# lauradarcy/gym-craftingworld

Measured on AMD Instinct MI355X. Metric: env-steps/sec at 65536 envs, 1/2/4/8 MI355X; bit-exact vs CPU ref, higher is better.
Workload: dtype u8; 1 GPU; BASELINE configs[2]: 65536 envs/GPU, 21x21 grid, full-frame 4x4-cell uint8 pixel obs, auto-reset, uniform random actions, max_steps=300; envs_per_gpu=65536, size=21, max_steps=300, obs_mode=pixels, raster=ray, task_lists=one (all nine tasks), launch=eager, episode_phases=synchronized start

## Files before the change

### gym_craftingworld_amd/csrc/cw_kernels.hip

```cpp
#include <hip/hip_runtime.h>
#include <stdint.h>

#include "cw_layout.h"
#include "cw_mt.h"

#define CW_WAVE 64
#define CW_BALLOT(p) __builtin_amdgcn_ballot_w64(p)
#define CW_ALT_FRAME_PACE 2

#ifdef CW_TRACE
__device__ unsigned long long cw_trace_buf[1024 * 8];
#define CW_STAMP(env, k) do { if (lane == 0) { cw_trace_buf[((env) & 1023) * 8 + (k)] = wall_clock64(); \
                                               if ((k) == 0 || (k) == 5) cw_trace_buf[((env) & 1023) * 8 + 6 + ((k) ? 1 : 0)] = clock64(); } } while (0)
extern "C" hipError_t cwk_trace_read(unsigned long long *dst) { return hipMemcpyFromSymbol(dst, HIP_SYMBOL(cw_trace_buf), sizeof(cw_trace_buf)); }
#else
#define CW_STAMP(env, k) do { } while (0)
#endif

enum { EMPTY = 0, STICKS = 1, AXE = 2, HAMMER = 3, ROCK = 4, TREE = 5, BREAD = 6, HOUSE = 7, WHEAT = 8 };
enum { T_MAKEBREAD = 0, T_EATBREAD = 1, T_BUILDHOUSE = 2, T_CHOPTREE = 3, T_CHOPROCK = 4,
       T_GOTOHOUSE = 5, T_MOVEAXE = 6, T_MOVEHAMMER = 7, T_MOVESTICKS = 8 };

typedef uint32_t u32x3 __attribute__((ext_vector_type(3)));
typedef u32x3 u32x3_a4 __attribute__((aligned(4)));
// ... 105 lines not shown
                                                bool whole)
{
    const uint32_t row_bytes = 9u * S;
    uint8_t *p = frame + (size_t)(3u * S) * row_bytes;
    if (whole) {
        for (uint32_t b = first; b < 3u * row_bytes; b += step) {
            const uint32_t x = b % row_bytes;
            p[b] = (hold != 0 && x >= 9u && x < 18u) ? 255 : 0;
        }
    } else {
        for (uint32_t j = first; j < 27u; j += step) p[(j / 9u) * row_bytes + 9u + (j % 9u)] = hold ? 255 : 0;
    }
}
__device__ __forceinline__ void render_frame_alt(uint8_t *__restrict__ dst0, uint8_t *__restrict__ dst1, int S, int ncell,
                                                 uint32_t div_magic, const uint32_t sp[8], uint32_t codes,
                                                 uint32_t agent_cell, uint32_t hold, int lane, int pace)
{
    const uint32_t row_bytes = 9u * S, FB = 27u * S * (uint32_t)(S + 1);
    uint32_t pos = 0xFFFFFFFFu, item = 0;
#pragma unroll
    for (int q = 0; q < 8; q++) {
        pos = (lane == q) ? sp[q] : pos;
        item = (lane == q) ? ((codes >> (4 * q)) & 15u) : item;
    }
    if (lane == 8) { pos = agent_cell; item = 9u; }
    if (lane == 9) { pos = agent_cell; item = hold; }
    uint32_t p_off = 0xFFFFFFFFu, p_val = 0;
    if (lane < 10 && item != 0 && pos < (uint32_t)ncell) {
        const uint32_t r = __umulhi(pos, div_magic), c = pos - r * S, k = item - 1u;
        const uint32_t k3 = (k >= 6u) ? 2u : (k >= 3u) ? 1u : 0u;
        p_off = (3u * r + k3) * row_bytes + 9u * c + 3u * (k - 3u * k3);
        p_val = cpv_color((int)k);
    } else if (lane >= 10 && lane < 19 && hold != 0) {
        const uint32_t j = (uint32_t)lane - 10u, jr = (j >= 6u) ? 2u : (j >= 3u) ? 1u : 0u;
        p_off = (3u * S + jr) * row_bytes + 9u + 3u * (j - 3u * jr);
        p_val = 0x00FFFFFFu;
    }
    const uint32_t held_off = __builtin_amdgcn_readlane(p_off, 9);
    const bool twice = lane < 8 && p_off != 0xFFFFFFFFu && p_off == held_off;
    if (twice) p_val = ((2u * (p_val & 0xFFu)) & 0xFFu) | ((2u * (p_val & 0xFF00u)) & 0xFF00u) | ((2u * (p_val & 0xFF0000u)) & 0xFF0000u);
    if (CW_BALLOT(twice) && lane == 9) p_off = 0xFFFFFFFFu;
    const bool p_any = p_off != 0xFFFFFFFFu;
    for (int which = 0; which < 2; which++) {
        uint8_t *const dst = which ? dst1 : dst0;
        if (!dst) break;
        const uint32_t head = (uint32_t)(-(intptr_t)dst) & 15u;
        const uint32_t n_body = (FB - head) >> 4;
        const uint32_t tail0 = head + 16u * n_body;
        if ((uint32_t)lane < head) dst[lane] = 0;
        if (tail0 + (uint32_t)lane < FB) dst[tail0 + lane] = 0;
        for (uint32_t j = (uint32_t)lane; j < n_body; j += CW_WAVE) {
            *(uint4 *)(dst + head + 16u * j) = make_uint4(0, 0, 0, 0);
            for (int z = 0; z < pace; z++) __builtin_amdgcn_s_sleep(1);
        }
        if (p_any) {
            dst[p_off] = (uint8_t)p_val;
            dst[p_off + 1] = (uint8_t)(p_val >> 8);
            dst[p_off + 2] = (uint8_t)(p_val >> 16);
        }
    }
}

__device__ __forceinline__ void render_frame(uint8_t *__restrict__ dst0, uint8_t *__restrict__ dst1,
                                             int S, int ncell, uint32_t div_magic, const uint32_t sp[8],
                                             const uint32_t rgb[8], uint32_t agent_cell, uint32_t hold_rgb,
                                             int lane)
{
    const uint32_t row_bytes = 12u * S;
    for (uint32_t cell = lane; cell < (uint32_t)ncell; cell += CW_WAVE) {
        const uint32_t r = __umulhi(cell, div_magic);
        const uint32_t c = cell - r * S;
        uint32_t col = 0;
#pragma unroll
        for (int k = 0; k < 8; k++) col = (cell == sp[k]) ? rgb[k] : col;
        const u32x3 d = cell_row_dwords(col);
        const bool ag = (cell == agent_cell);
        const u32x3 d1 = ag ? overlay_dwords(d, 0x00FFFFFFu) : d;
        const u32x3 d2 = ag ? overlay_dwords(d, hold_rgb) : d;
        const size_t off = (size_t)(4u * r) * row_bytes + 12u * c;
        uint8_t *q = dst0 + off;
        *(u32x3_a4 *)(q) = d;
        *(u32x3_a4 *)(q + row_bytes) = d1;
        *(u32x3_a4 *)(q + 2 * row_bytes) = d2;
        *(u32x3_a4 *)(q + 3 * row_bytes) = d;
        if (dst1) {
            uint8_t *q1 = dst1 + off;
            *(u32x3_a4 *)(q1) = d;
            *(u32x3_a4 *)(q1 + row_bytes) = d1;
            *(u32x3_a4 *)(q1 + 2 * row_bytes) = d2;
            *(u32x3_a4 *)(q1 + 3 * row_bytes) = d;
        }
    }
}
__device__ __forceinline__ void paint_state_frame(const CwParams &P, uint8_t *dst, const uint32_t sp[8], uint32_t codes, uint32_t agent_cell,
                                                  uint32_t hold, int lane, uint8_t *dst1 = nullptr)
{
    if (P.raster == 1) {
        render_frame_alt(dst, dst1, P.size, P.ncell, P.div_magic, sp, codes, agent_cell, hold, lane, CW_ALT_FRAME_PACE);
    } else {
        uint32_t rgb[8];
#pragma unroll
        for (int k = 0; k < 8; k++) rgb[k] = rgb_of_code((codes >> (4 * k)) & 15u);
        render_frame(dst, dst1, P.size, P.ncell, P.div_magic, sp, rgb, agent_cell, hold ? rgb_of_code(hold) : 0x00FFFFFFu, lane);
    }
}
__device__ __forceinline__ uint32_t agent_cell_of(const CwParams &P, uint32_t hx) { return (hx & 0xFFu) * P.size + ((hx >> 8) & 0xFFu); }
__device__ __forceinline__ uint32_t hold_of(uint32_t hx) { return (hx >> 16) & 0xFFu; }
enum { CW_SRC_CURRENT = 0, CW_SRC_INIT = 1, CW_SRC_GOAL = 2 };
__device__ __forceinline__ void load_state_uniform(const CwParams &P, int env, int src, uint32_t sp[8], uint32_t &codes, uint32_t &agent_cell, uint32_t &hold)
{
    uint4 v_p;
    uint32_t v_c, v_a, v_h = 0;
    if (src == CW_SRC_CURRENT) {
        const uint4 h = P.hdr[env];
        v_p = P.pos[env];
        v_c = h.w;
        v_a = agent_cell_of(P, h.x);
        v_h = hold_of(h.x);
    } else if (src == CW_SRC_INIT) {
        v_p = P.init_pos[env];
        v_c = CW_CODES_INITIAL;
        v_a = P.init_agent[env];
    } else {
        v_p = P.goal_pos[env];
        v_c = P.goal_codes[env];
        v_a = P.goal_agent[env];
    }
    unpack_pos(make_uint4(__builtin_amdgcn_readfirstlane(v_p.x), __builtin_amdgcn_readfirstlane(v_p.y), __builtin_amdgcn_readfirstlane(v_p.z),
                          __builtin_amdgcn_readfirstlane(v_p.w)), sp);
    codes = __builtin_amdgcn_readfirstlane(v_c);
    agent_cell = __builtin_amdgcn_readfirstlane(v_a);
    hold = __builtin_amdgcn_readfirstlane(v_h);
}

struct CwStepOut {
    int reward;
    bool done, success, invalid, changed;
    uint32_t dirty0, dirty1;
    bool mark0, mark1;
    uint32_t step_num, achieved, desired;
    uint32_t n_success;
};

__device__ __forceinline__ int32_t episode_return_of(const CwParams &P, const CwStepOut &o)
{
    return (int32_t)o.n_success * (P.max_steps + 1) - (int32_t)o.step_num;
}

template <typename InitPosFn>
__device__ __forceinline__ CwStepOut step_env(const CwParams &P, uint4 &h, uint32_t sp[8], int a, InitPosFn load_init_pos)
{
    CwStepOut o;
    const int S = P.size;
    int ar = h.x & 0xFF, ac = (h.x >> 8) & 0xFF;
    uint32_t hold = (h.x >> 16) & 0xFF;
    uint32_t achieved = h.y & 0xFFFFu;
    const uint32_t desired = h.y >> 16;
    const uint32_t step_num = min((h.z & 0xFFFFu) + 1u, 0xFFFFu);
    const uint32_t flags = (h.z >> 16) & ~CW_FLAG_RESET;
    uint32_t codes = h.w;

    o.invalid = (unsigned)a > 5u;
    bool changed = false;
    const uint32_t cell = ar * S + ac;
    const int idx_here = slot_at(sp, cell);
    const uint32_t code_here = code_of(codes, idx_here);
    o.dirty0 = cell;
    o.dirty1 = 0xFFFFFFFFu;
    o.mark0 = o.mark1 = false;

    if (a == 4) {
        if (code_here >= STICKS && code_here <= HAMMER && hold == 0) {
            hold = code_here;
#pragma unroll
            for (int k = 0; k < 8; k++) sp[k] = (k == idx_here) ? CW_POS_HELD : sp[k];
            changed = true;
        }
    } else if (a == 5) {
        if (hold != 0 && idx_here < 0) {
#pragma unroll
            for (int k = 0; k < 8; k++) sp[k] = (sp[k] == CW_POS_HELD) ? cell : sp[k];
            hold = 0;
            changed = true;
        }
    } else if (!o.invalid) {
        const int dr = (a == 0) ? -1 : (a == 2) ? 1 : 0;
        const int dc = (a == 1) ? 1 : (a == 3) ? -1 : 0;
        const int nr = min(max(ar + dr, 0), S - 1);
        const int nc = min(max(ac + dc, 0), S - 1);
        uint32_t old_obj = 0;
        uint32_t cur_code = code_here;
        if (nr != ar || nc != ac) {
            const uint32_t ncell = nr * S + nc;
            const int idx_t = slot_at(sp, ncell);
            const uint32_t t = code_of(codes, idx_t);
            const bool cant = (t == ROCK && hold != 3) || (t == TREE && hold != 2);
            if (!cant) {
                changed = true;
                o.dirty1 = ncell;
                o.mark0 = true;
                ar = nr; ac = nc;
                old_obj = t;
                uint32_t nw = t;
                if (t == ROCK || t == BREAD) nw = EMPTY;
                else if (t == TREE) nw = STICKS;
                else if (t == STICKS && hold == 3) nw = HOUSE;
                else if (t == WHEAT && hold == 2) nw = BREAD;
                if (nw != t) {
                    codes = (codes & ~(15u << (4 * idx_t))) | (nw << (4 * idx_t));
                    if (nw == EMPTY) {
#pragma unroll
                        for (int k = 0; k < 8; k++) sp[k] = (k == idx_t) ? CW_POS_GONE : sp[k];
                    }
                }
                cur_code = nw;
                o.mark1 = nw == t;
            }
        }
        const uint32_t pcell = ar * S + ac;
        if (old_obj == BREAD) achieved |= 1u << T_EATBREAD;
        else if (old_obj == ROCK) achieved |= 1u << T_CHOPROCK;
        else if (old_obj == TREE) achieved |= 1u << T_CHOPTREE;
        achieved = (cur_code == HOUSE) ? (achieved | (1u << T_GOTOHOUSE))
                                       : (achieved & ~(1u << T_GOTOHOUSE));
        if (hold != 0) {
            const uint4 ip = load_init_pos();
            const uint32_t ip_sticks = ip.x & 0xFFFFu, ip_axe = ip.x >> 16;
            const uint32_t ip_hammer = ip.y & 0xFFFFu, ip_tree = ip.z & 0xFFFFu;
            if (hold == 1) {
                const bool home = (pcell == ip_sticks) ||
                                  (pcell == ip_tree && (achieved & (1u << T_CHOPTREE)));
                achieved = home ? (achieved & ~(1u << T_MOVESTICKS)) : (achieved | (1u << T_MOVESTICKS));
            } else if (hold == 2) {
                if (old_obj == WHEAT) achieved |= 1u << T_MAKEBREAD;
                achieved = (pcell == ip_axe) ? (achieved & ~(1u << T_MOVEAXE)) : (achieved | (1u << T_MOVEAXE));
            } else {
                if (old_obj == STICKS) achieved |= 1u << T_BUILDHOUSE;
                achieved = (pcell == ip_hammer) ? (achieved & ~(1u << T_MOVEHAMMER)) : (achieved | (1u << T_MOVEHAMMER));
            }
        }
    }

    int reward = -1;
    if (changed) {
        const uint32_t am = achieved & P.task_mask, dm = desired & P.task_mask;
        bool hit;
        if (flags & CW_FLAG_SUBSET)
            hit = ((dm & ~am) == 0) && (((~(dm ^ am)) & P.task_mask) != 0);
        else
            hit = (am == dm);
        reward = hit ? P.max_steps : -1;
    }
    o.reward = reward;
    o.changed = changed;
    o.success = (reward == P.max_steps);
    o.done = (step_num >= (uint32_t)P.max_steps) || o.success;
    o.step_num = step_num;
    o.achieved = achieved;
    o.desired = desired;
    o.n_success = min((flags >> 2) + (o.success ? 1u : 0u), 0x3FFFu);

    h.x = (uint32_t)ar | ((uint32_t)ac << 8) | (hold << 16) | (h.x & 0xFF000000u);
    h.y = achieved | (desired << 16);
    h.z = step_num | (((flags & 3u) | (o.n_success << 2)) << 16);
    h.w = codes;
    return o;
}

__device__ __forceinline__ void paint_changed_cells(const CwParams &P, int env, const uint4 &h, const uint32_t sp[8], const CwStepOut &o)
{
    uint8_t *frame = P.obs + (size_t)env * P.frame_bytes;
    const uint32_t hold = hold_of(h.x);
    const uint32_t acell = agent_cell_of(P, h.x);
    if (P.raster == 1) {
        const uint32_t r0 = __umulhi(o.dirty0, P.div_magic);
        alt_paint_tile(frame, P.size, r0, o.dirty0 - r0 * P.size, code_of(h.w, slot_at(sp, o.dirty0)), o.dirty0 == acell, hold);
        if (o.dirty1 != 0xFFFFFFFFu) {
            const uint32_t r1 = __umulhi(o.dirty1, P.div_magic);
            alt_paint_tile(frame, P.size, r1, o.dirty1 - r1 * P.size, code_of(h.w, slot_at(sp, o.dirty1)), o.dirty1 == acell, hold);
        }
        alt_paint_strip(frame, P.size, hold, 0, 1, false);
    } else {
        paint_cell(frame, P.size, o.dirty0, code_of(h.w, slot_at(sp, o.dirty0)), o.dirty0 == acell, hold, P.div_magic, o.mark0);
        if (o.dirty1 != 0xFFFFFFFFu)
            paint_cell(frame, P.size, o.dirty1, code_of(h.w, slot_at(sp, o.dirty1)), o.dirty1 == acell, hold, P.div_magic, o.mark1);
    }
}

__device__ __forceinline__ void store_step_outputs(const CwParams &P, int env, const CwStepOut &o)
{
    P.reward[env] = o.reward;
    P.done[env] = o.done ? 1 : 0;
    P.achieved_out[env] = (uint16_t)o.achieved;
    P.desired_out[env] = (uint16_t)o.desired;
    if (o.done) { P.episode_length[env] = (int32_t)o.step_num; P.episode_return[env] = episode_return_of(P, o); }
}

__device__ __forceinline__ int load_action(const void *actions, int act_dtype, int i)
{
    if (act_dtype == 0) return ((const int32_t *)actions)[i];
    if (act_dtype == 1) { const long long a = ((const long long *)actions)[i]; return a == (long long)(int)a ? (int)a : -1; }
    return ((const uint8_t *)actions)[i];
}

struct CwGoalState { uint4 pos; uint32_t codes, agent; };
__device__ __forceinline__ bool pop_next_episode(const CwParams &P, int env, uint32_t ctl, uint4 &h, uint32_t sp[8], bool count_episode, CwGoalState *goal = nullptr)
{
    const uint32_t slot = ctl & 0xFFu;
    const size_t at = (size_t)slot * P.n_envs + env;
    const uint4 m = P.nx_misc[at];
    const uint4 ipos = P.nx_init_pos[at];
    const uint4 gpos = P.nx_goal_pos[at];
    const int32_t ep_no = count_episode ? P.ep_no[env] : 0;
    if (!(m.z >> 31)) return false;
    P.init_pos[env] = ipos;
    P.goal_pos[env] = gpos;
    if (goal) { goal->pos = gpos; goal->codes = m.y; goal->agent = m.x >> 16; }
    P.goal_codes[env] = m.y;
    P.init_agent[env] = (uint16_t)(m.x & 0xFFFFu);
    P.goal_agent[env] = (uint16_t)(m.x >> 16);
    if (count_episode) P.ep_no[env] = ep_no + 1;
    ((uint32_t *)(P.nx_misc + at))[2] = 0;
    P.nx_ctl[env] = (slot + 1u == CW_LA_DEPTH ? 0u : slot + 1u) | CW_CTL_QUEUED;
    const uint32_t ia = m.x & 0xFFFFu;
    const uint32_t ar = __umulhi(ia, P.div_magic), ac = ia - ar * P.size;
    h.x = ar | (ac << 8) | (h.x & 0xFF000000u);
    h.y = (m.z & 0xFFFFu) << 16;
    h.z = (CW_FLAG_RESET | (((m.z >> 16) & 1u) ? CW_FLAG_SUBSET : 0u)) << 16;
    h.w = CW_CODES_INITIAL;
    unpack_pos(ipos, sp);
    return true;
}

__device__ __forceinline__ void note_slow_reset(const CwParams &P, int env, uint32_t ctl)
{
    atomicAdd(&P.counters[5], 1ull);
    if (!(ctl & CW_CTL_QUEUED)) P.nx_ctl[env] = ctl | CW_CTL_QUEUED;
}

__global__ __launch_bounds__(256) void cw_step_kernel(CwParams P, const void *actions, int act_dtype, int paint_dirty)
{
    const int i = blockIdx.x * blockDim.x + threadIdx.x;
    if (i == 0) {
        atomicAdd(&P.counters[0], (unsigned long long)P.n_envs);
    }
    const bool live = i < P.n_envs;
    bool done = false, success = false, invalid = false;
    if (live) {
        const int a = load_action(actions, act_dtype, i);
        uint4 h = P.hdr[i];
        uint32_t sp[8];
        unpack_pos(P.pos[i], sp);
        const CwStepOut o = step_env(P, h, sp, a, [&]() { return P.init_pos[i]; });
        done = o.done; success = o.success; invalid = o.invalid;

        P.hdr[i] = h;
        P.pos[i] = pack_pos(sp);
        store_step_outputs(P, i, o);
        if (paint_dirty && o.changed) paint_changed_cells(P, i, h, sp, o);
    }
    const unsigned long long m_done = CW_BALLOT(done), m_succ = CW_BALLOT(success), m_inv = CW_BALLOT(invalid);
    if ((m_done | m_inv) && (threadIdx.x & (CW_WAVE - 1)) == 0) {
        if (m_done) atomicAdd(&P.counters[1], (unsigned long long)__popcll(m_done));
        if (m_succ) atomicAdd(&P.counters[2], (unsigned long long)__popcll(m_succ));
        if (m_inv) atomicAdd(&P.counters[3], (unsigned long long)__popcll(m_inv));
    }
}


__device__ __forceinline__ uint32_t shuffle_tokens(CwMtWave &mt, int n)
{
    const uint32_t lane = mt.lane;
    uint32_t hit = 0;
    uint32_t v_tok = 0;
    int i = n - 1;

    while (i >= 10) {
        if (mt.used == 64) mt.gen();
        const int take = min(64 - mt.used, i - 8);
        const uint32_t d = mt.v_out;
        const unsigned long long valid = (~0ull >> (64 - take)) << mt.used;
        unsigned long long acc = CW_BALLOT((d & (0xFFFFFFFFu >> __builtin_clz((uint32_t)i))) <= (uint32_t)i) & valid;
        uint32_t i_l = 0, v_l = 0;
        for (;;) {
            const uint32_t before = __builtin_amdgcn_mbcnt_hi((uint32_t)(acc >> 32),
                                                              __builtin_amdgcn_mbcnt_lo((uint32_t)acc, 0u));
            i_l = (uint32_t)i - before;
            v_l = d & (0xFFFFFFFFu >> __builtin_clz(i_l));
            const unsigned long long acc2 = CW_BALLOT(v_l <= i_l) & valid;
            if (acc2 == acc) break;
            acc = acc2;
        }
        unsigned long long ev = CW_BALLOT(v_l <= 8u && !((hit >> (v_l & 15u)) & 1u)) & acc;
        while (ev) {
            const int l = __builtin_ctzll(ev);
            ev &= ev - 1;
            const uint32_t vv = __builtin_amdgcn_readlane(v_l, l);
            const uint32_t il = __builtin_amdgcn_readlane(i_l, l);
            if (!((hit >> vv) & 1u)) v_tok = (lane == vv) ? il : v_tok;
            hit |= 1u << vv;
        }
        i -= __popcll(acc);
        mt.used += take;
    }
    unsigned long long low = 0;
#pragma unroll
    for (int q = 0; q < 9; q++) low |= (unsigned long long)(((hit >> q) & 1u) ? 15u : (uint32_t)q) << (4 * q);

    while (i >= 1) {
        const uint32_t mask = 0xFFFFFFFFu >> __builtin_clz((uint32_t)i);
        const uint32_t v = mt.next() & mask;
        if (v <= (uint32_t)i) {
            const uint32_t b = (v <= 8u) ? (uint32_t)((low >> (4u * v)) & 15ull) : 15u;
            const uint32_t a = (i <= 8) ? (uint32_t)((low >> (4u * i)) & 15ull) : 15u;
            if (b != 15u) v_tok = (lane == b) ? (uint32_t)i : v_tok;
            if (v <= 8u) low = (low & ~(15ull << (4u * v))) | ((unsigned long long)a << (4u * v));
            i--;
        }
// ... 197 lines not shown
    const int n_waves = (int)gridDim.x * CW_RESET_WAVES;
    for (int env = (int)blockIdx.x * CW_RESET_WAVES + wave_in_block; env < P.n_envs; env += n_waves) {
        const uint4 v_h = P.hdr[env];
        const uint32_t menu_id = __builtin_amdgcn_readfirstlane(v_h.x) >> 24;
        const bool count_episode = (__builtin_amdgcn_readfirstlane(v_h.z) & 0xFFFFu) != 0;
        const uint32_t ctl = P.lookahead ? __builtin_amdgcn_readfirstlane(P.nx_ctl[env]) : 0u;
        if (P.lookahead && (__builtin_amdgcn_readfirstlane(P.nx_misc[(size_t)(ctl & 0xFFu) * P.n_envs + env].z) >> 31)) {
            if (lane == 0) {
                uint4 h = v_h;
                uint32_t sp[8];
                pop_next_episode(P, env, ctl, h, sp, count_episode);
                P.pos[env] = pack_pos(sp);
                P.hdr[env] = h;
                P.achieved_out[env] = 0;
                P.desired_out[env] = (uint16_t)(h.y >> 16);
            }
            continue;
        }
        const CwResetOut r = reset_env_wave(P, env, [&]() { return menu_id; }, s_mt[wave_in_block], lane);
        if (lane == 0) {
            store_episode_records(P, env, r, count_episode);
            P.pos[env] = r.init_pos;
            P.hdr[env] = reset_header(P, r, menu_id);
            P.achieved_out[env] = 0;
            P.desired_out[env] = (uint16_t)r.desired;
        }
    }
}

template <bool PAINT>
__global__ __launch_bounds__(CW_RESET_WAVES *CW_WAVE) void cw_reset_masked_kernel(CwParams P, const uint8_t *__restrict__ mask, int epb)
{
    __shared__ uint32_t s_mt[CW_RESET_WAVES][CW_MT_WORDS];
    const int lane = threadIdx.x & (CW_WAVE - 1);
    const int wave_in_block = __builtin_amdgcn_readfirstlane(threadIdx.x / CW_WAVE);
    for (int base = (int)blockIdx.x * epb; base < P.n_envs; base += (int)gridDim.x * epb) {
        const int mine = base + lane;
        const bool in_chunk = lane < epb && mine < P.n_envs;
        const uint32_t v_sel = in_chunk ? (uint32_t)mask[mine] : 0u;
        unsigned long long m = CW_BALLOT(v_sel != 0u);
        for (int rank = 0; m; rank++) {
            const int l = __builtin_ctzll(m);
            m &= m - 1;
            if ((rank & (CW_RESET_WAVES - 1)) != wave_in_block) continue;
            const int env = base + l;
            const uint4 v_h = P.hdr[env];
            const uint32_t menu_id = __builtin_amdgcn_readfirstlane(v_h.x) >> 24;
            const bool count_episode = (__builtin_amdgcn_readfirstlane(v_h.z) & 0xFFFFu) != 0;
            const uint32_t ctl = P.lookahead ? __builtin_amdgcn_readfirstlane(P.nx_ctl[env]) : 0u;
            uint4 ipos, gpos;
            uint32_t iagent, gagent, gcodes;
            if (P.lookahead && (__builtin_amdgcn_readfirstlane(P.nx_misc[(size_t)(ctl & 0xFFu) * P.n_envs + env].z) >> 31)) {
                uint4 h = v_h;
                uint32_t sp[8] = {0, 0, 0, 0, 0, 0, 0, 0};
                CwGoalState goal;
                goal.pos = make_uint4(0, 0, 0, 0); goal.codes = 0; goal.agent = 0;
                if (lane == 0) {
                    pop_next_episode(P, env, ctl, h, sp, count_episode, PAINT ? &goal : nullptr);
                    P.pos[env] = pack_pos(sp);
                    P.hdr[env] = h;
                    P.achieved_out[env] = 0;
                    P.desired_out[env] = (uint16_t)(h.y >> 16);
                }
                if constexpr (PAINT) {
                    const uint4 p0 = pack_pos(sp);
                    ipos = make_uint4(__builtin_amdgcn_readfirstlane(p0.x), __builtin_amdgcn_readfirstlane(p0.y), __builtin_amdgcn_readfirstlane(p0.z),
                                      __builtin_amdgcn_readfirstlane(p0.w));
                    gpos = make_uint4(__builtin_amdgcn_readfirstlane(goal.pos.x), __builtin_amdgcn_readfirstlane(goal.pos.y),
                                      __builtin_amdgcn_readfirstlane(goal.pos.z), __builtin_amdgcn_readfirstlane(goal.pos.w));
                    iagent = agent_cell_of(P, __builtin_amdgcn_readfirstlane(h.x));
                    gagent = __builtin_amdgcn_readfirstlane(goal.agent);
                    gcodes = __builtin_amdgcn_readfirstlane(goal.codes);
                }
            } else {
                const CwResetOut r = reset_env_wave(P, env, [&]() { return menu_id; }, s_mt[wave_in_block], lane);
                if (lane == 0) {
                    store_episode_records(P, env, r, count_episode);
                    P.pos[env] = r.init_pos;
                    P.hdr[env] = reset_header(P, r, menu_id);
                    P.achieved_out[env] = 0;
                    P.desired_out[env] = (uint16_t)r.desired;
                    if (P.lookahead) note_slow_reset(P, env, ctl);
                }
                ipos = r.init_pos; gpos = r.goal_pos;
                iagent = r.init_agent; gagent = r.goal_agent; gcodes = r.goal_codes;
            }
            if constexpr (PAINT) {
                const size_t off = (size_t)env * P.frame_bytes;
                uint32_t jp[8];
                unpack_pos(ipos, jp);
                paint_state_frame(P, P.init_img + off, jp, CW_CODES_INITIAL, iagent, 0u, lane, P.obs + off);
                unpack_pos(gpos, jp);
                paint_state_frame(P, P.desired_img + off, jp, gcodes, gagent, 0u, lane);
            } else {
                (void)ipos; (void)gpos; (void)iagent; (void)gagent; (void)gcodes;
            }
        }
    }
}

__global__ __launch_bounds__(CW_RESET_WAVES *CW_WAVE) void cw_refill_kernel(CwParams P, int all_envs)
{
    __shared__ uint32_t s_mt[CW_RESET_WAVES][CW_MT_WORDS];
    const int lane = threadIdx.x & (CW_WAVE - 1);
    const int wave_in_block = __builtin_amdgcn_readfirstlane(threadIdx.x / CW_WAVE);
    const int wave = blockIdx.x * CW_RESET_WAVES + wave_in_block;
    const int n_waves = gridDim.x * CW_RESET_WAVES;
    if (P.la_feedback && blockIdx.x == 0 && threadIdx.x == 0)
        __hip_atomic_store(P.la_feedback, P.counters[5], __ATOMIC_RELAXED, __HIP_MEMORY_SCOPE_SYSTEM);
    enum { CHUNK = 16 };
    for (int base = wave * CHUNK; base < P.n_envs; base += n_waves * CHUNK) {
        const int mine = base + lane;
        const uint32_t v_ctl = (lane < CHUNK && mine < P.n_envs) ? P.nx_ctl[mine] : 0u;
        unsigned long long m = CW_BALLOT(lane < CHUNK && mine < P.n_envs && (all_envs || (v_ctl & CW_CTL_QUEUED)));
        while (m) {
            const int l = __builtin_ctzll(m);
            m &= m - 1;
            const int env = base + l;
            const uint32_t ctl = __builtin_amdgcn_readlane(v_ctl, l);
            const uint32_t v_hx = P.hdr[env].x;
            const uint32_t head = ctl & 0xFFu;
            for (uint32_t k = 0; k < CW_LA_DEPTH; k++) {
                const uint32_t slot = head + k >= CW_LA_DEPTH ? head + k - CW_LA_DEPTH : head + k;
                if (__builtin_amdgcn_readfirstlane(P.nx_misc[(size_t)slot * P.n_envs + env].z) >> 31) continue;
                const CwResetOut r = reset_env_wave(P, env, [&]() { return __builtin_amdgcn_readfirstlane(v_hx) >> 24; }, s_mt[wave_in_block], lane);
                if (lane == 0) store_next_record(P, env, (int)slot, r);
            }
            if ((ctl & CW_CTL_QUEUED) && lane == 0) P.nx_ctl[env] = head;
        }
    }
}

__global__ __launch_bounds__(CW_RESET_WAVES *CW_WAVE) void cw_rollout_kernel(CwParams P, const uint8_t *actions, int T,
                                                                             int32_t *rewards, uint8_t *dones, int epw)
{
    __shared__ uint32_t s_mt[CW_RESET_WAVES][CW_MT_WORDS];
    const int lane = threadIdx.x & (CW_WAVE - 1);
    const int wave_in_block = __builtin_amdgcn_readfirstlane(threadIdx.x / CW_WAVE);
    const int wave = blockIdx.x * CW_RESET_WAVES + wave_in_block;
    const int env0 = wave * epw;
    if (env0 >= P.n_envs) return;
    const int env = env0 + lane;
    const bool live = lane < epw && env < P.n_envs;
    const int e = live ? env : env0;
    uint4 h = P.hdr[e];
    uint32_t sp[8];
    unpack_pos(P.pos[e], sp);
    uint4 ip = P.init_pos[e];
    uint32_t ctl = P.lookahead ? P.nx_ctl[e] : 0u;
    unsigned long long n_done = 0, n_succ = 0, n_inv = 0;
    int reward = -1;
    bool done = false;
    uint32_t achieved = 0, desired = 0, step_num = 0;
    for (int t = 0; t < T; t++) {
        const int a = actions[(size_t)t * P.n_envs + e];
        const CwStepOut o = step_env(P, h, sp, a, [&]() { return ip; });
        reward = o.reward; done = o.done; achieved = o.achieved; desired = o.desired; step_num = o.step_num;
        if (live) {
            if (rewards) rewards[(size_t)t * P.n_envs + env] = o.reward;
            if (dones) dones[(size_t)t * P.n_envs + env] = o.done ? 1 : 0;
        }
        const unsigned long long m_all = CW_BALLOT(live && o.done);
        n_done += __popcll(m_all);
        n_succ += __popcll(CW_BALLOT(live && o.success));
        n_inv += __popcll(CW_BALLOT(live && o.invalid));
        if (m_all && live && o.done) { P.episode_length[env] = (int32_t)o.step_num; P.episode_return[env] = episode_return_of(P, o); }
        bool popped = false;
        const uint32_t ctl_was = ctl;
        if (live && o.done && P.lookahead) {
            popped = pop_next_episode(P, env, ctl, h, sp, true);
            if (popped) { ip = pack_pos(sp); ctl = ((ctl & 0xFFu) + 1u == CW_LA_DEPTH ? 0u : (ctl & 0xFFu) + 1u) | CW_CTL_QUEUED; }
        }
        const unsigned long long m_pop = CW_BALLOT(popped);
        unsigned long long m = m_all & ~m_pop;
        while (m) {
            const int l = __builtin_ctzll(m);
            m &= m - 1;
            const int env_l = env0 + l;
            const uint32_t menu_id = __builtin_amdgcn_readlane(h.x, l) >> 24;
            const CwResetOut r = reset_env_wave(P, env_l, [&]() { return menu_id; }, s_mt[wave_in_block], lane);
            if (lane == 0) {
                store_episode_records(P, env_l, r, true);
                if (P.lookahead) note_slow_reset(P, env_l, __builtin_amdgcn_readlane(ctl_was, l));
            }
            if (lane == l) {
                h = reset_header(P, r, menu_id);
                unpack_pos(r.init_pos, sp);
                ip = r.init_pos;
                ctl |= CW_CTL_QUEUED;
            }
        }
    }
    if (live) {
        P.hdr[env] = h;
        P.pos[env] = pack_pos(sp);
        P.reward[env] = reward;
        P.done[env] = done ? 1 : 0;
        P.achieved_out[env] = (uint16_t)achieved;
        P.desired_out[env] = (uint16_t)desired;
        (void)step_num;
    }
    if (lane == 0) {
        atomicAdd(&P.counters[0], (unsigned long long)min(epw, P.n_envs - env0) * (unsigned long long)T);
        if (n_done) atomicAdd(&P.counters[1], n_done);
        if (n_succ) atomicAdd(&P.counters[2], n_succ);
        if (n_inv) atomicAdd(&P.counters[3], n_inv);
    }
}

__global__ __launch_bounds__(CW_WAVE) void cw_resident_kernel(CwParams P, CwResident *R, uint32_t seq0, int paint_dirty,
                                                              unsigned long long idle_ticks, unsigned long long life_ticks)
{
    const int lane = threadIdx.x;
    uint4 h = P.hdr[0];
    uint32_t sp[8];
    unpack_pos(P.pos[0], sp);
    const uint4 ip = P.init_pos[0];
    uint32_t last = seq0;
    const unsigned long long t_start = wall_clock64();
    unsigned long long t_last = t_start;
    uint32_t reason = 0;
    for (;;) {
        const unsigned long long bell = __hip_atomic_load(&R->bell, __ATOMIC_ACQUIRE, __HIP_MEMORY_SCOPE_SYSTEM);
        const uint32_t d = (uint32_t)bell;
        const uint32_t seq = d >> 8;
        if (seq != last) {
            if (lane == 0) {
                const int a = (int)(d & 0x7Fu);
                const CwStepOut o = step_env(P, h, sp, a, [&]() { return ip; });
                P.hdr[0] = h;
                P.pos[0] = pack_pos(sp);
                store_step_outputs(P, 0, o);
                if (paint_dirty && o.changed) paint_changed_cells(P, 0, h, sp, o);
                atomicAdd(&P.counters[0], 1ull);
                if (o.done) atomicAdd(&P.counters[1], 1ull);
                if (o.success) atomicAdd(&P.counters[2], 1ull);
                if (o.invalid) atomicAdd(&P.counters[3], 1ull);
            }
            if (P.res_onehot && (d & 0x80u)) {
                const uint32_t hx = __builtin_amdgcn_readlane(h.x, 0), codes = __builtin_amdgcn_readlane(h.w, 0);
                uint32_t bp[8];
#pragma unroll
                for (int k = 0; k < 8; k++) bp[k] = __builtin_amdgcn_readlane(sp[k], 0);
                const uint32_t agent_cell = agent_cell_of(P, hx), hold = hold_of(hx);
                for (int cell = lane; cell < P.ncell; cell += CW_WAVE) {
                    const uint32_t code = code_of(codes, slot_at(bp, (uint32_t)cell));
                    uint32_t bits = code ? (1u << (code - 1)) : 0u;
                    if ((uint32_t)cell == agent_cell) bits |= (1u << 8) | (hold ? (1u << (8 + hold)) : 0u);
                    *(u32x3_a4 *)(P.res_onehot + 12 * cell) = onehot_dwords(bits);
                }
            }
            __threadfence_system();
            if (lane == 0) __hip_atomic_store(&R->ack, seq, __ATOMIC_RELEASE, __HIP_MEMORY_SCOPE_SYSTEM);
            last = seq;
            t_last = wall_clock64();
            continue;
        }
        const unsigned long long now = wall_clock64();
        if (bell >> 32) { reason = 1; break; }
        if (now - t_last > idle_ticks) { reason = 2; break; }
        if (now - t_start > life_ticks) { reason = 3; break; }
    }
    if (lane == 0) __hip_atomic_store(&R->exited, reason | (last << 8), __ATOMIC_RELEASE, __HIP_MEMORY_SCOPE_SYSTEM);
}

struct CwPaintJob { uint4 pos; uint32_t codes, agent_hold_kind, env, pad; };
enum { CW_JOB_INIT = 0, CW_JOB_GOAL = 1, CW_JOB_TERMINAL = 2 };
template <int PAINT, bool TERM>
__device__ __forceinline__ void fused_step(const CwParams &P, const void *actions, int act_dtype, int epw, int wave, uint32_t *s_mt_wave,
                                           CwPaintJob *s_jobs, int *s_njobs, int *s_cnt )
{
    constexpr int paint = PAINT;
    const int lane = threadIdx.x & (CW_WAVE - 1);
    const int wave_in_block = __builtin_amdgcn_readfirstlane(threadIdx.x / CW_WAVE);
    const int env0 = wave * epw;
    const bool wave_live = env0 < P.n_envs;
    const int env = env0 + lane;
    const bool live = wave_live && lane < epw && env < P.n_envs;
    const int e = live ? env : (wave_live ? env0 : 0);
    const int a = load_action(actions, act_dtype, e);
    uint4 h = P.hdr[e];
    uint32_t sp[8];
    unpack_pos(P.pos[e], sp);
    const uint4 ip = P.init_pos[e];
    const uint32_t ctl = P.lookahead ? P.nx_ctl[e] : 0u;
    if (threadIdx.x == 0) { *s_njobs = 0; s_cnt[0] = s_cnt[1] = s_cnt[2] = 0; }
    __syncthreads();
    const CwStepOut o = step_env(P, h, sp, a, [&]() { return ip; });
    const bool done = live && o.done;
    if (live) {
        store_step_outputs(P, env, o);
        if constexpr (PAINT == 1) { if (o.changed && !o.done) paint_changed_cells(P, env, h, sp, o); }
    }
    const uint4 h_last = h;
    uint32_t sp_last[8];
    if constexpr (TERM) {
#pragma unroll
        for (int k = 0; k < 8; k++) sp_last[k] = sp[k];
    }
    const unsigned long long m_all = CW_BALLOT(done);
    const unsigned long long m_succ = CW_BALLOT(live && o.success);
    const unsigned long long m_inv = CW_BALLOT(live && o.invalid);
    if (lane == 0 && (m_all | m_inv)) {
        if (m_all) atomicAdd(&s_cnt[0], (int)__popcll(m_all));
        if (m_succ) atomicAdd(&s_cnt[1], (int)__popcll(m_succ));
        if (m_inv) atomicAdd(&s_cnt[2], (int)__popcll(m_inv));
    }
    bool popped = false;
    CwGoalState goal;
    goal.pos = make_uint4(0, 0, 0, 0); goal.codes = 0; goal.agent = 0;
    if (done && P.lookahead) popped = pop_next_episode(P, env, ctl, h, sp, true, PAINT != 0 ? &goal : nullptr);
    const unsigned long long m_pop = CW_BALLOT(popped);
    __syncthreads();
    if (threadIdx.x == 0) {
        if (blockIdx.x == 0) atomicAdd(&P.counters[0], (unsigned long long)P.n_envs);
        if (s_cnt[0]) atomicAdd(&P.counters[1], (unsigned long long)s_cnt[0]);
        if (s_cnt[1]) atomicAdd(&P.counters[2], (unsigned long long)s_cnt[1]);
        if (s_cnt[2]) atomicAdd(&P.counters[3], (unsigned long long)s_cnt[2]);
    }
    constexpr int jpe = TERM ? 3 : 2;
    int jmine = 0;
    if constexpr (PAINT != 0) {
        int jbase = 0;
        if (m_all) {
            if (lane == 0) jbase = atomicAdd(s_njobs, jpe * __popcll(m_all));
            jbase = __shfl(jbase, 0);
        }
        jmine = jbase + jpe * __popcll(m_all & ((1ull << lane) - 1ull));
        if constexpr (TERM) if (done) {
            CwPaintJob &j = s_jobs[jmine + 2];
            j.pos = pack_pos(sp_last);
            j.codes = h_last.w;
            j.agent_hold_kind = agent_cell_of(P, h_last.x) | (hold_of(h_last.x) << 16) | (CW_JOB_TERMINAL << 24);
// ... 761 lines not shown
```

Baseline: 312.3 million env-steps/s.

## Make step_env branch-free and prefetch next action in fused step loop

Rewrites the per-env step logic as straight-line predicated code: both candidate cells are looked up unconditionally, and the position, code and achieved updates become select-based with a single slot-rewrite loop. The aim is to remove wave divergence from random actions, since different lanes take the pick, drop or move paths. The fused loop also software-prefetches the next step's action byte. An empty asm barrier keeps the lane index in a VGPR for the reset call. The cost is that every lane now does the work of every branch, and the init_pos lookup always runs.

```diff
diff --git a/gym_craftingworld_amd/csrc/cw_kernels.hip b/gym_craftingworld_amd/csrc/cw_kernels.hip
--- a/gym_craftingworld_amd/csrc/cw_kernels.hip
+++ b/gym_craftingworld_amd/csrc/cw_kernels.hip
@@ -281,118 +281,83 @@
 {
     CwStepOut o;
     const int S = P.size;
-    int ar = h.x & 0xFF, ac = (h.x >> 8) & 0xFF;
-    uint32_t hold = (h.x >> 16) & 0xFF;
-    uint32_t achieved = h.y & 0xFFFFu;
+    const uint4 ip = load_init_pos();
+    const int ar = h.x & 0xFF, ac = (h.x >> 8) & 0xFF;
+    const uint32_t hold = (h.x >> 16) & 0xFF;
+    const uint32_t achieved = h.y & 0xFFFFu;
     const uint32_t desired = h.y >> 16;
     const uint32_t step_num = min((h.z & 0xFFFFu) + 1u, 0xFFFFu);
     const uint32_t flags = (h.z >> 16) & ~CW_FLAG_RESET;
-    uint32_t codes = h.w;
-
+    const uint32_t codes = h.w;
+
+    const bool is_move = (unsigned)a < 4u, is_pick = a == 4, is_drop = a == 5;
     o.invalid = (unsigned)a > 5u;
-    bool changed = false;
-    const uint32_t cell = ar * S + ac;
-    const int idx_here = slot_at(sp, cell);
-    const uint32_t code_here = code_of(codes, idx_here);
+    const int dr = (is_move && !(a & 1)) ? a - 1 : 0;
+    const int dc = (is_move && (a & 1)) ? 2 - a : 0;
+    const int nr = min(max(ar + dr, 0), S - 1);
+    const int nc = min(max(ac + dc, 0), S - 1);
+    const uint32_t cell = ar * S + ac, ncell = nr * S + nc;
+    const int idx_here = slot_at(sp, cell), idx_t = slot_at(sp, ncell);
+    const uint32_t code_here = code_of(codes, idx_here), t = code_of(codes, idx_t);
+
+    const bool can_pick = is_pick && hold == 0 && code_here - STICKS <= (uint32_t)(HAMMER - STICKS);
+    const bool can_drop = is_drop && hold != 0 && idx_here < 0;
+    const bool cant = (t == ROCK && hold != 3) || (t == TREE && hold != 2);
+    const bool moved = ncell != cell && !cant;
+    const bool eaten = t == ROCK || t == BREAD;
+    uint32_t nw = eaten ? (uint32_t)EMPTY : t;
+    nw = (t == TREE) ? (uint32_t)STICKS : nw;
+    nw = (t == STICKS && hold == 3) ? (uint32_t)HOUSE : nw;
+    nw = (t == WHEAT && hold == 2) ? (uint32_t)BREAD : nw;
+    const uint32_t old_obj = moved ? t : 0u;
+    const uint32_t cur_code = moved ? nw : code_here;
+    const bool changed = can_pick || can_drop || moved;
+
+    const uint32_t from = can_pick ? cell : can_drop ? CW_POS_HELD : (moved && eaten) ? ncell : 0xFFFFFFFFu;
+    const uint32_t to = can_pick ? CW_POS_HELD : can_drop ? cell : CW_POS_GONE;
+#pragma unroll
+    for (int k = 0; k < 8; k++) sp[k] = (sp[k] == from) ? to : sp[k];
+    const uint32_t codes_new = codes ^ ((moved ? (nw ^ t) : 0u) << ((4 * idx_t) & 28));
+    const uint32_t hold_new = can_pick ? code_here : can_drop ? 0u : hold;
+    const uint32_t ar_new = moved ? nr : ar, ac_new = moved ? nc : ac;
+    const uint32_t pcell = moved ? ncell : cell;
     o.dirty0 = cell;
-    o.dirty1 = 0xFFFFFFFFu;
-    o.mark0 = o.mark1 = false;
-
-    if (a == 4) {
-        if (code_here >= STICKS && code_here <= HAMMER && hold == 0) {
-            hold = code_here;
-#pragma unroll
-            for (int k = 0; k < 8; k++) sp[k] = (k == idx_here) ? CW_POS_HELD : sp[k];
-            changed = true;
-        }
-    } else if (a == 5) {
-        if (hold != 0 && idx_here < 0) {
-#pragma unroll
-            for (int k = 0; k < 8; k++) sp[k] = (sp[k] == CW_POS_HELD) ? cell : sp[k];
-            hold = 0;
-            changed = true;
-        }
-    } else if (!o.invalid) {
-        const int dr = (a == 0) ? -1 : (a == 2) ? 1 : 0;
-        const int dc = (a == 1) ? 1 : (a == 3) ? -1 : 0;
-        const int nr = min(max(ar + dr, 0), S - 1);
-        const int nc = min(max(ac + dc, 0), S - 1);
-        uint32_t old_obj = 0;
-        uint32_t cur_code = code_here;
-        if (nr != ar || nc != ac) {
-            const uint32_t ncell = nr * S + nc;
-            const int idx_t = slot_at(sp, ncell);
-            const uint32_t t = code_of(codes, idx_t);
-            const bool cant = (t == ROCK && hold != 3) || (t == TREE && hold != 2);
-            if (!cant) {
-                changed = true;
-                o.dirty1 = ncell;
-                o.mark0 = true;
-                ar = nr; ac = nc;
-                old_obj = t;
-                uint32_t nw = t;
-                if (t == ROCK || t == BREAD) nw = EMPTY;
-                else if (t == TREE) nw = STICKS;
-                else if (t == STICKS && hold == 3) nw = HOUSE;
-                else if (t == WHEAT && hold == 2) nw = BREAD;
-                if (nw != t) {
-                    codes = (codes & ~(15u << (4 * idx_t))) | (nw << (4 * idx_t));
-                    if (nw == EMPTY) {
-#pragma unroll
-                        for (int k = 0; k < 8; k++) sp[k] = (k == idx_t) ? CW_POS_GONE : sp[k];
-                    }
-                }
-                cur_code = nw;
-                o.mark1 = nw == t;
-            }
-        }
-        const uint32_t pcell = ar * S + ac;
-        if (old_obj == BREAD) achieved |= 1u << T_EATBREAD;
-        else if (old_obj == ROCK) achieved |= 1u << T_CHOPROCK;
-        else if (old_obj == TREE) achieved |= 1u << T_CHOPTREE;
-        achieved = (cur_code == HOUSE) ? (achieved | (1u << T_GOTOHOUSE))
-                                       : (achieved & ~(1u << T_GOTOHOUSE));
-        if (hold != 0) {
-            const uint4 ip = load_init_pos();
-            const uint32_t ip_sticks = ip.x & 0xFFFFu, ip_axe = ip.x >> 16;
-            const uint32_t ip_hammer = ip.y & 0xFFFFu, ip_tree = ip.z & 0xFFFFu;
-            if (hold == 1) {
-                const bool home = (pcell == ip_sticks) ||
-                                  (pcell == ip_tree && (achieved & (1u << T_CHOPTREE)));
-                achieved = home ? (achieved & ~(1u << T_MOVESTICKS)) : (achieved | (1u << T_MOVESTICKS));
-            } else if (hold == 2) {
-                if (old_obj == WHEAT) achieved |= 1u << T_MAKEBREAD;
-                achieved = (pcell == ip_axe) ? (achieved & ~(1u << T_MOVEAXE)) : (achieved | (1u << T_MOVEAXE));
-            } else {
-                if (old_obj == STICKS) achieved |= 1u << T_BUILDHOUSE;
-                achieved = (pcell == ip_hammer) ? (achieved & ~(1u << T_MOVEHAMMER)) : (achieved | (1u << T_MOVEHAMMER));
-            }
-        }
-    }
-
-    int reward = -1;
-    if (changed) {
-        const uint32_t am = achieved & P.task_mask, dm = desired & P.task_mask;
-        bool hit;
-        if (flags & CW_FLAG_SUBSET)
-            hit = ((dm & ~am) == 0) && (((~(dm ^ am)) & P.task_mask) != 0);
-        else
-            hit = (am == dm);
-        reward = hit ? P.max_steps : -1;
-    }
-    o.reward = reward;
+    o.dirty1 = moved ? ncell : 0xFFFFFFFFu;
+    o.mark0 = moved;
+    o.mark1 = moved && nw == t;
+
+    uint32_t ach = achieved;
+    ach |= (old_obj == BREAD) ? 1u << T_EATBREAD : 0u;
+    ach |= (old_obj == ROCK) ? 1u << T_CHOPROCK : 0u;
+    ach |= (old_obj == TREE) ? 1u << T_CHOPTREE : 0u;
+    ach |= (old_obj == WHEAT && hold == 2) ? 1u << T_MAKEBREAD : 0u;
+    ach |= (old_obj == STICKS && hold >= 3) ? 1u << T_BUILDHOUSE : 0u;
+    ach = (cur_code == HOUSE) ? (ach | (1u << T_GOTOHOUSE)) : (ach & ~(1u << T_GOTOHOUSE));
+    const uint32_t ip_sticks = ip.x & 0xFFFFu, ip_axe = ip.x >> 16;
+    const uint32_t ip_hammer = ip.y & 0xFFFFu, ip_tree = ip.z & 0xFFFFu;
+    const uint32_t ip_own = (hold == 1) ? ip_sticks : (hold == 2) ? ip_axe : ip_hammer;
+    const bool home = (pcell == ip_own) || (hold == 1 && pcell == ip_tree && (ach & (1u << T_CHOPTREE)));
+    const uint32_t away = (hold == 0) ? 0u : (hold == 1) ? 1u << T_MOVESTICKS : (hold == 2) ? 1u << T_MOVEAXE : 1u << T_MOVEHAMMER;
+    ach = (ach & ~away) | (home ? 0u : away);
+    const uint32_t achieved_new = is_move ? ach : achieved;
+
+    const uint32_t am = achieved_new & P.task_mask, dm = desired & P.task_mask;
+    const bool hit_subset = ((dm & ~am) == 0) && (((~(dm ^ am)) & P.task_mask) != 0);
+    const bool subset = (flags & CW_FLAG_SUBSET) != 0;
+    const bool hit = (subset && hit_subset) || (!subset && am == dm);
+    o.success = changed && hit;
+    o.reward = o.success ? P.max_steps : -1;
     o.changed = changed;
-    o.success = (reward == P.max_steps);
     o.done = (step_num >= (uint32_t)P.max_steps) || o.success;
     o.step_num = step_num;
-    o.achieved = achieved;
+    o.achieved = achieved_new;
     o.desired = desired;
     o.n_success = min((flags >> 2) + (o.success ? 1u : 0u), 0x3FFFu);
 
-    h.x = (uint32_t)ar | ((uint32_t)ac << 8) | (hold << 16) | (h.x & 0xFF000000u);
-    h.y = achieved | (desired << 16);
+    h.x = ar_new | (ac_new << 8) | (hold_new << 16) | (h.x & 0xFF000000u);
+    h.y = achieved_new | (desired << 16);
     h.z = step_num | (((flags & 3u) | (o.n_success << 2)) << 16);
-    h.w = codes;
+    h.w = codes_new;
     return o;
 }
 
@@ -896,8 +861,12 @@
     int reward = -1;
     bool done = false;
     uint32_t achieved = 0, desired = 0, step_num = 0;
+    const uint8_t *act = actions + e;
+    int a_next = T > 0 ? act[0] : 0;
     for (int t = 0; t < T; t++) {
-        const int a = actions[(size_t)t * P.n_envs + e];
+        const int a = a_next;
+        act += P.n_envs;
+        if (t + 1 < T) a_next = *act;
         const CwStepOut o = step_env(P, h, sp, a, [&]() { return ip; });
         reward = o.reward; done = o.done; achieved = o.achieved; desired = o.desired; step_num = o.step_num;
         if (live) {
@@ -922,7 +891,9 @@
             m &= m - 1;
             const int env_l = env0 + l;
             const uint32_t menu_id = __builtin_amdgcn_readlane(h.x, l) >> 24;
-            const CwResetOut r = reset_env_wave(P, env_l, [&]() { return menu_id; }, s_mt[wave_in_block], lane);
+            int lane_r = lane;
+            asm volatile("" : "+v"(lane_r));
+            const CwResetOut r = reset_env_wave(P, env_l, [&]() { return menu_id; }, s_mt[wave_in_block], lane_r);
             if (lane == 0) {
                 store_episode_records(P, env_l, r, true);
                 if (P.lookahead) note_slow_reset(P, env_l, __builtin_amdgcn_readlane(ctl_was, l));
```

Result: no change. 314.9 million env-steps/s, median of 5 (+0.8%).
